# IMMachinations/Task-Vector-Replication

Hardware: AMD Instinct MI355X
Metric: patched-forward prompts/sec, Pythia-2.8B layer×head CIE sweep, 1–8 GPUs (higher is better)
Workload: dtype f32 (x2f16 emulation: fp32 activations as 2 fp16 planes against the checkpoint's exact fp16 weights, 2 MFMA products, fp32 accumulate); 1 GPU; pythia-2.8b CIE sweep 32x32 sites, 12 prompts/step, 4-shot, T=15, fp16-valued weights (exact-fp16 GEMMs, 2 products); parallelism=single GPU, gemm=x2f16, weights=fp16, exact16_gemms=True

## Files before the change

### task-vector-replication_amd/csrc/gemm_pingpong.hpp

```cpp
#pragma once
#include <hip/hip_runtime.h>
#include <stdint.h>

#include <type_traits>

#include "gemm_planar.hpp"

namespace tvr {

constexpr int PP_THREADS = 512;
constexpr int PP_TILE_ELEMS = 256 * 256;

inline int gemm_pingpong_grid(int M, int N) { return ((M + 255) / 256) * ((N + 255) / 256); }

__host__ __device__ inline void pp_tile_coords(int wg, int nbm, int nbn, int& m0, int& n0, int gm = GEMM_GROUP_M) {
  const int per_group = gm * nbn;
  const int grp = wg / per_group;
  const int first_m = grp * gm;
  const int gsz = nbm - first_m < gm ? nbm - first_m : gm;
  const int in_grp = wg - grp * per_group;
  m0 = (first_m + in_grp % gsz) * 256;
  n0 = (in_grp / gsz) * 256;
}

constexpr int PP_EPI_LDR = 260;
#ifndef TVR_PP_NT
#define TVR_PP_NT 1
#endif
constexpr bool PP_NT_STORES = TVR_PP_NT;
#ifndef TVR_PP_SLICE_MIN_K
#define TVR_PP_SLICE_MIN_K 16384
#endif
constexpr int PP_SLICE_MIN_K = TVR_PP_SLICE_MIN_K;
#ifndef TVR_PP_SLICE_FORM
#define TVR_PP_SLICE_FORM 2
#endif
#ifndef TVR_PP_SLICE_FORM_WX
#define TVR_PP_SLICE_FORM_WX 2
#endif
#ifndef TVR_PP_WX_STAGE
#define TVR_PP_WX_STAGE 0
#endif
#ifndef TVR_PP_WX_WIDE
#define TVR_PP_WX_WIDE 2
#endif
#ifndef TVR_PP_BF16_WIDE
#define TVR_PP_BF16_WIDE 0
#endif
#ifndef TVR_PP_WX_2PHASE
#define TVR_PP_WX_2PHASE 0
#endif
#ifndef TVR_PP_PF
#define TVR_PP_PF 1
#endif
__device__ __forceinline__ f32x4 slice_add(f32x4 c, f32x4 t) { return c + t; }
constexpr int PP_EPI_LDS = 128 * PP_EPI_LDR * 2;

template <int CTRL>
__device__ __forceinline__ float dpp_f(float v) {
  return __int_as_float(__builtin_amdgcn_update_dpp(0, __float_as_int(v), CTRL, 0xF, 0xF, false));
}
template <int CTRL>
__device__ __forceinline__ int dpp_i(int v) {
  return __builtin_amdgcn_update_dpp(0, v, CTRL, 0xF, 0xF, false);
}
constexpr int DPP_QUAD_X1 = 0xB1, DPP_QUAD_X2 = 0x4E;
__device__ __forceinline__ void quad_argmax(float& bv, int& bi) {
  argmax_merge(bv, bi, dpp_f<DPP_QUAD_X1>(bv), dpp_i<DPP_QUAD_X1>(bi));
  argmax_merge(bv, bi, dpp_f<DPP_QUAD_X2>(bv), dpp_i<DPP_QUAD_X2>(bi));
}
__device__ __forceinline__ void pp_stats_rows(const GemmEpi& ep, const float* L, int grow0, int col0, int rows,
                                              int Nlim, int t, float acc_scale) {
  const int r = t >> 2, q = t & 3;
  if (r >= rows) return;
  Nlim = min(Nlim, 256);
  const int K = ep.stats_k, rec = 2 + 2 * K, tile = col0 >> 8;
  const float* Lr = L + r * PP_EPI_LDR;
  const float* bias = ep.bias ? ep.bias + col0 : nullptr;
  auto elem = [&](float a, float b) { return __fadd_rn(__fmul_rn(a, acc_scale), b); };
  auto chunk = [&](int i) {
    const int c = 16 * i + 4 * q;
    const f32x4 a = *(const f32x4*)(Lr + c);
    const f32x4 b = bias ? *(const f32x4*)(bias + c) : f32x4{0.f, 0.f, 0.f, 0.f};
    return f32x4{elem(a[0], b[0]), elem(a[1], b[1]), elem(a[2], b[2]), elem(a[3], b[3])};
  };
  const int nc = (Nlim - 4 * q + 15) >> 4;
  float mx = -INFINITY;
#pragma unroll 2
  for (int i = 0; i < nc; ++i) {
    const f32x4 v = chunk(i);
    mx = fmaxf(mx, fmaxf(fmaxf(v[0], v[1]), fmaxf(v[2], v[3])));
  }
  mx = fmaxf(mx, dpp_f<DPP_QUAD_X1>(mx));
  mx = fmaxf(mx, dpp_f<DPP_QUAD_X2>(mx));
  float se = 0.f, bv = -INFINITY;
  int bi = 0x7fffffff;
#pragma unroll 2
  for (int i = 0; i < nc; ++i) {
    const f32x4 v = chunk(i);
    se += (expf(v[0] - mx) + expf(v[1] - mx)) + (expf(v[2] - mx) + expf(v[3] - mx));
#pragma unroll
    for (int e = 0; e < 4; ++e)
      if (v[e] > bv) {
        bv = v[e];
        bi = col0 + 16 * i + 4 * q + e;
      }
  }
  se += dpp_f<DPP_QUAD_X1>(se);
  se += dpp_f<DPP_QUAD_X2>(se);
  const int m = grow0 + r;
  float* o = ep.stats + ((size_t)m * ep.stats_tiles + tile) * rec;
  if (q == 0) {
    o[0] = mx;
    o[1] = se;
    if (ep.targets && ep.tlogit) {
      const int tc = ep.targets[m] - col0;
      if (tc >= 0 && tc < Nlim) ep.tlogit[m] = elem(Lr[tc], bias ? bias[tc] : 0.f);
    }
  }
  for (int j = 0; j < K; ++j) {
    if (j > 0) {
      const float pv = bv;
      const int pi = bi;
      bv = -INFINITY;
      bi = 0x7fffffff;
#pragma unroll 2
  for (int i = 0; i < nc; ++i) {
        const f32x4 v = chunk(i);
#pragma unroll
        for (int e = 0; e < 4; ++e) {
          const int c = col0 + 16 * i + 4 * q + e;
          if ((v[e] < pv || (v[e] == pv && c > pi)) && v[e] > bv) {
            bv = v[e];
            bi = c;
          }
        }
      }
    }
    quad_argmax(bv, bi);
    if (q == 0) {
      o[2 + j] = bv;
      o[2 + K + j] = __int_as_float(bi);
    }
  }
}

template <int EPI, int FMT, bool NOSTORE = false, int TM = 8, int TN = 4>
__device__ __forceinline__ void pp_epilogue_lds(const GemmEpi& ep, const f32x4 (&acc)[TM][TN], float* L, int row0,
                                                int col0, int Mlim, int Nlim, int wr, int wc, int lane, int t,
                                                float acc_scale) {
  static_assert((TM == 8 && TN == 4) || (TM == 4 && TN == 8), "wave tile 128 x 64 or 64 x 128");
  bool split8 = false;
  if constexpr (EPI == EPI_SPLIT_GELU_ACT) split8 = col0 >= ep.n_split && Nlim >= 256;
  float range_mx = 0.f;
  const int c8 = (t & 31) * 8, c4 = (t & 63) * 4;
  float b8[8];
  f32x4 b4 = {0.f, 0.f, 0.f, 0.f};
  if (split8) {
#pragma unroll
    for (int k = 0; k < 8; ++k) b8[k] = ep.bias ? ep.bias[col0 + c8 + k] : 0.f;
  } else if (EPI != EPI_STATS && ep.bias && c4 < Nlim) {
#pragma unroll
    for (int k = 0; k < 4; ++k) b4[k] = ep.bias[col0 + c4 + k];
  }
#pragma unroll
  for (int p = 0; p < 2; ++p) {
    if ((TM == 8 ? wr : wr >> 1) == p) {
      const int r0 = TM == 8 ? 0 : (wr & 1) * 64;
#pragma unroll
      for (int i = 0; i < TM; ++i)
#pragma unroll
        for (int j = 0; j < TN; ++j)
          *(f32x4*)(L + (r0 + i * 16 + (lane & 15)) * PP_EPI_LDR + wc * (16 * TN) + j * 16 + 4 * (lane >> 4)) =
              EPI == EPI_STATS ? acc[i][j] : acc[i][j] * acc_scale;
    }
    __syncthreads();
    const int rows = min(128, Mlim - p * 128);
    if constexpr (EPI == EPI_STATS) {
      pp_stats_rows(ep, L, row0 + p * 128, col0, rows, Nlim, t, acc_scale);
    } else if (split8) {
      constexpr int RPT = 128 / (PP_THREADS / 32);
      const int rb = t >> 5;
      int orow[RPT];
#pragma unroll
      for (int i = 0; i < RPT; ++i) orow[i] = row0 + p * 128 + min(rb + i * (PP_THREADS / 32), max(rows - 1, 0));
      if (ep.out_rows) {
#pragma unroll
        for (int i = 0; i < RPT; ++i) orow[i] = ep.out_rows[orow[i]];
      }
#pragma unroll
      for (int i = 0; i < RPT; ++i) {
        const int r = rb + i * (PP_THREADS / 32);
        if (r >= rows) break;
        const float* src = L + r * PP_EPI_LDR + c8;
        const f32x4 x0 = *(const f32x4*)src, x1 = *(const f32x4*)(src + 4);
        float v[8] = {x0[0] + b8[0], x0[1] + b8[1], x0[2] + b8[2], x0[3] + b8[3],
                      x1[0] + b8[4], x1[1] + b8[5], x1[2] + b8[6], x1[3] + b8[7]};
        const int m = row0 + p * 128 + r;
        if (ep.raw && m < ep.raw_rows) {
          float* q = ep.raw + (size_t)m * ep.ld_raw + (col0 + c8 - ep.n_split);
          *(f32x4*)q = f32x4{v[0], v[1], v[2], v[3]};
          *(f32x4*)(q + 4) = f32x4{v[4], v[5], v[6], v[7]};
        }
#pragma unroll
        for (int k = 0; k < 8; k += 2) {
          const f32x2 g = gelu_erf2(f32x2{v[k], v[k + 1]});
          v[k] = g.x;
          v[k + 1] = g.y;
        }
        if (!NOSTORE || v[0] == 1.2345e-30f)
          store_act8<FMT, PP_NT_STORES>(ep.out1h + (size_t)orow[i] * ep.ld1h + act_col<FMT>(col0 + c8 - ep.n_split),
                                        act_ps<FMT>(ep.ps1h), v,
                                        ep.range_flag, &range_mx);
      }
    } else if (c4 < Nlim) {
      constexpr int RB = 8, NB = 128 / (PP_THREADS / 64) / RB;
      const int rb = t >> 6;
#pragma unroll
      for (int b = 0; b < NB; ++b) {
        int orow[RB];
        f32x4 rr[RB];
#pragma unroll
        for (int i = 0; i < RB; ++i) orow[i] = row0 + p * 128 + min(rb + (b * RB + i) * (PP_THREADS / 64), max(rows - 1, 0));
        if (ep.out_rows) {
#pragma unroll
          for (int i = 0; i < RB; ++i) orow[i] = ep.out_rows[orow[i]];
        }
        if constexpr (EPI == EPI_RESID) {
#pragma unroll
          for (int i = 0; i < RB; ++i) rr[i] = *(const f32x4*)(ep.resid + (size_t)orow[i] * ep.ldr + col0 + c4);
        }
#pragma unroll
        for (int i = 0; i < RB; ++i) {
          const int r = rb + (b * RB + i) * (PP_THREADS / 64);
          if (r >= rows) break;
          f32x4 v = *(const f32x4*)(L + r * PP_EPI_LDR + c4) + b4;
          if (!NOSTORE || v[0] == 1.2345e-30f) {
            if constexpr (EPI == EPI_RESID)
              st16<false>(ep.out0 + (size_t)orow[i] * ep.ld0 + col0 + c4, v + rr[i]);
            else
              epi_store4<EPI, FMT, PP_NT_STORES && EPI == EPI_SPLIT_GELU_ACT>(ep, orow[i], col0 + c4, v);
          }
        }
      }
    }
    __syncthreads();
  }
  if constexpr (EPI == EPI_SPLIT_GELU_ACT && act_is_x2(FMT))
    if (range_mx >= X2_FP16_OVERFLOW && ep.range_flag) atomicOr(ep.range_flag, 1u);
}

template <int FMT>
struct PpLds {
  using F = PlanarFmt<FMT>;
  static constexpr int BUF = 2 * F::NPL * 256 * F::BK;
  static constexpr int HALVES = (2 * BUF + 512) > PP_EPI_LDS ? (2 * BUF + 512) : PP_EPI_LDS;
};

template <int EPI, int FMT, bool VEC, int VAR, bool SL, bool WX = false, bool PFOK = true, bool AIL = false>
__device__ __forceinline__ void pp_tile(const uint16_t* __restrict__ A, int lda, size_t aps,
                                        const uint16_t* __restrict__ W, int ldw, size_t wps, float acc_scale, int M,
                                        int N, const GemmEpi& ep, int m0, int n0, int kbeg, int nk, float* part, int has_part,
                                        unsigned long long st0, unsigned long long sr0) {
  using F = PlanarFmt<FMT>;
  using frag = typename F::frag;
  constexpr int NPL = F::NPL, BK = F::BK, KG = BK / 32;
  constexpr int CPR = BK / 8;
  constexpr int RPP = 64 / CPR;
  constexpr int PPP = 128 / RPP;
  constexpr int PL = 256 * BK;
  static_assert(!WX || FMT == ACT_X2F16, "one-plane weights: x2f16 activations only");
  constexpr int WNPL = WX ? 1 : NPL;
  constexpr int BUF = (NPL + WNPL) * PL;
  constexpr bool P2 = WX && !SL && TVR_PP_WX_2PHASE;
  constexpr int NBUF = P2 ? 3 : 2;
  constexpr int DUMMY = NBUF * BUF;
  constexpr int LDS_HALVES = P2 ? (NBUF * BUF + 512 > PP_EPI_LDS ? NBUF * BUF + 512 : PP_EPI_LDS)
                                : PpLds<FMT>::HALVES;
  static_assert(LDS_HALVES * 2 <= 160 * 1024, "LDS budget (P2)");
  static_assert(NPL * KG == 2, "two fragments per 16-row slice per k-tile");
  static_assert(PpLds<FMT>::HALVES * 2 <= 160 * 1024, "LDS budget");
  static_assert(!AIL || FMT == ACT_X2F16, "the interleaved A layout is an x2f16 form");
  constexpr int ACPR = AIL ? 8 : CPR;
  constexpr int ARPP = 64 / ACPR;
  constexpr int ABK = ACPR * 8;
  constexpr int OFMT = AIL ? (int)ACT_X2F16I : FMT;
  __shared__ __attribute__((aligned(16))) uint16_t lds[LDS_HALVES];

  int t = threadIdx.x;
  asm volatile("" : "+v"(t));
  const int wave = t >> 6, lane = t & 63;
  const int wr = wave >> 2, wc = wave & 3;

  const int wave_s = __builtin_amdgcn_readfirstlane(wave);
  const uint16_t* Ab = ep.a2 != nullptr && n0 >= ep.a2_col ? ep.a2 : A;
  const uint16_t* src[4][2];
  int dst[4][2];
#pragma unroll
  for (int R = 0; R < 4; ++R) {
#pragma unroll
    for (int s = 0; s < 2; ++s) {
      const int pi = (WX && R >= 2) ? wave_s : 2 * wave_s + s;
      const bool ail = AIL && R < 2;
      const int plane = ail ? 0 : pi / PPP;
      const int x0 = ail ? pi * ARPP : (pi % PPP) * RPP;
      int trow0;
      if (R < 2)
        trow0 = ((x0 >> 6) << 7) + (x0 & 63) + 64 * R;
      else
        trow0 = ((x0 >> 5) << 6) + (x0 & 31) + 32 * (R - 2);
      const int row = trow0 + (ail ? lane / ACPR : lane / CPR);
      const int chunk = ail ? (lane % ACPR) ^ planar_g<ACPR>(row) : (lane % CPR) ^ planar_g<CPR>(row);
      if (R < 2) {
        const int am = min(m0 + row, M - 1);
        src[R][s] = Ab + plane * aps + (size_t)(ep.a_rows ? ep.a_rows[am] : am) * lda + chunk * 8;
        dst[R][s] = plane * PL + trow0 * (AIL ? ABK : BK);
      } else {
        src[R][s] = W + plane * wps + (size_t)min(n0 + row, N - 1) * ldw + chunk * 8;
        dst[R][s] = (NPL + plane) * PL + trow0 * BK;
      }
    }
  }
  auto stage = [&](int R, int kt) {
    if (VAR == 1 && kt >= 2) return;
    const bool live = kt < nk;
    const int koff = live && VAR != 12 ? (kbeg + kt) * (AIL && R < 2 ? ABK : BK) : 0;
    const int boff = (P2 ? kt % 3 : kt & 1) * BUF;
#pragma unroll
    for (int s = 0; s < ((WX && R >= 2) ? 1 : 2); ++s) glds16(src[R][s] + koff, lds + (live ? boff + dst[R][s] : DUMMY));
  };

  int aoff[2], boff[2];
#pragma unroll
  for (int f = 0; f < 2; ++f) {
    const int p = NPL == 2 ? f : 0, g = NPL == 2 ? 0 : f;
    const int ra = wr * 128 + (lane & 15), rb = wc * 64 + (lane & 15);
    const int c = 4 * g + (lane >> 4);
    if constexpr (AIL)
      aoff[f] = ra * ABK + (((4 * f + (lane >> 4)) ^ planar_g<ACPR>(ra)) << 3);
    else
      aoff[f] = p * PL + ra * BK + ((c ^ planar_g<CPR>(ra)) << 3);
    boff[f] = (NPL + p) * PL + rb * BK + ((c ^ planar_g<CPR>(rb)) << 3);
  }

  f32x4 acc[8][4];
#pragma unroll
  for (int i = 0; i < 8; ++i)
#pragma unroll
    for (int j = 0; j < 4; ++j) acc[i][j] = f32x4{};
  frag fa[4][2], fwl[2][2], fwh[2][2];
  constexpr bool PF = PFOK && ((TVR_PP_PF != 0) != (VAR == 21)) && !P2 && !WX && !(FMT == ACT_X2F16 && SL);
  [[maybe_unused]] frag fx[2][2];

  const int vi = __builtin_amdgcn_readfirstlane(min(8, max(0, (M - m0 - wr * 128 + 15) >> 4)));
  auto read_a = [&](const uint16_t* base, int i0, auto part, int ifirst = 0) {
#pragma unroll
    for (int i = 0; i < 4; ++i)
      if (i >= ifirst && (!decltype(part)::value || i0 + i < vi))
#pragma unroll
        for (int f = 0; f < 2; ++f) fa[i][f] = *(const frag*)(base + aoff[f] + (i0 + i) * 16 * ABK);
  };
  auto read_fx = [&](const uint16_t* base, auto part) {
#pragma unroll
    for (int i = 0; i < 2; ++i)
      if (!decltype(part)::value || i < vi)
#pragma unroll
        for (int f = 0; f < 2; ++f) fx[i][f] = *(const frag*)(base + aoff[f] + i * 16 * ABK);
  };
  auto read_w = [&](const uint16_t* base, int j0, frag (&fw)[2][2], auto part) {
    if (decltype(part)::value && vi == 0) return;
#pragma unroll
    for (int j = 0; j < 2; ++j)
#pragma unroll
      for (int f = 0; f < (WX ? 1 : 2); ++f) fw[j][f] = *(const frag*)(base + boff[f] + (j0 + j) * 16 * BK);
  };
  [[maybe_unused]] f32x4 tc[2] = {f32x4{0.f, 0.f, 0.f, 0.f}, f32x4{0.f, 0.f, 0.f, 0.f}};
  auto mfma_quadrant = [&](int i0, int j0, const frag (&fw)[2][2], auto part, int ci, int cj) {
#if TVR_PP_SLICE_FORM_WX >= 1
    if constexpr (FMT == ACT_X2F16 && SL && WX && !decltype(part)::value) {
      f32x4 t[4][2];
#pragma unroll
      for (int i = 0; i < 4; ++i) {
        const int di = i == 0 ? ci : i0 + i - 1, dj = i == 0 ? cj : j0;
#pragma unroll
        for (int q = 0; q < 4; ++q) {
          const int j = TVR_PP_SLICE_FORM_WX == 2 ? (q & 1) : (q >> 1), pz = TVR_PP_SLICE_FORM_WX == 2 ? (q >> 1) : (q & 1);
          t[i][j] = __builtin_amdgcn_mfma_f32_16x16x32_f16(fw[j][0], fa[i][pz == 0 ? 1 : 0],
                                                             pz == 0 ? f32x4{0.f, 0.f, 0.f, 0.f} : t[i][j], 0, 0, 0);
          __builtin_amdgcn_sched_group_barrier(0x008, 1, 0);
#pragma unroll
          for (int e = 2 * q; e < 2 * q + 2; ++e)
            acc[di][dj + (e >> 2)][e & 3] += i == 0 ? tc[e >> 2][e & 3] : t[i - 1][e >> 2][e & 3];
          __builtin_amdgcn_sched_group_barrier(0x002, 2, 0);
        }
      }
      tc[0] = t[3][0];
      tc[1] = t[3][1];
      return;
    }
#endif
    if constexpr (FMT == ACT_X2F16 && SL && !WX && !decltype(part)::value) {
#if TVR_PP_SLICE_FORM >= 1
      f32x4 t[4][2];
#pragma unroll
      for (int i = 0; i < 4; ++i) {
        const int di = i == 0 ? ci : i0 + i - 1, dj = i == 0 ? cj : j0;
#pragma unroll
        for (int q = 0; q < 6; ++q) {
          const int j = q & 1, p = q >> 1;
          t[i][j] = __builtin_amdgcn_mfma_f32_16x16x32_f16(fw[j][p == 1 ? 1 : 0], fa[i][p == 0 ? 1 : 0],
                                                             p == 0 ? f32x4{0.f, 0.f, 0.f, 0.f} : t[i][j], 0, 0, 0);
          __builtin_amdgcn_sched_group_barrier(0x008, 1, 0);
#if TVR_PP_SLICE_FORM == 2
          const int e0 = q < 2 ? 0 : 2 * (q - 2), e1 = q < 2 ? 0 : 2 * (q - 2) + 2;
#else
          const int e0 = q < 2 ? 2 * q : q + 2, e1 = q < 2 ? 2 * q + 2 : q + 3;
#endif
#pragma unroll
          for (int e = e0; e < e1; ++e)
            acc[di][dj + (e >> 2)][e & 3] += i == 0 ? tc[e >> 2][e & 3] : t[i - 1][e >> 2][e & 3];
          if (e1 - e0 == 2)
            __builtin_amdgcn_sched_group_barrier(0x002, 2, 0);
          else if (e1 - e0 == 1)
            __builtin_amdgcn_sched_group_barrier(0x002, 1, 0);
        }
      }
      tc[0] = t[3][0];
      tc[1] = t[3][1];
      return;
#else
      (void)ci;
      (void)cj;
      f32x4 t[4][2];
#pragma unroll
      for (int i = 0; i <= 4; ++i) {
        if (i < 4) {
#pragma unroll
          for (int j = 0; j < 2; ++j)
            t[i][j] = __builtin_amdgcn_mfma_f32_16x16x32_f16(fw[j][0], fa[i][1], f32x4{0.f, 0.f, 0.f, 0.f}, 0, 0, 0);
#pragma unroll
          for (int j = 0; j < 2; ++j) t[i][j] = __builtin_amdgcn_mfma_f32_16x16x32_f16(fw[j][1], fa[i][0], t[i][j], 0, 0, 0);
#pragma unroll
          for (int j = 0; j < 2; ++j) t[i][j] = __builtin_amdgcn_mfma_f32_16x16x32_f16(fw[j][0], fa[i][0], t[i][j], 0, 0, 0);
          __builtin_amdgcn_sched_group_barrier(0x008, 6, 0);
        }
        if (i > 0) {
#pragma unroll
          for (int j = 0; j < 2; ++j) acc[i0 + i - 1][j0 + j] = slice_add(acc[i0 + i - 1][j0 + j], t[i - 1][j]);
          __builtin_amdgcn_sched_group_barrier(0x002, 5, 0);
        }
      }
      return;
#endif
    }
#pragma unroll
    for (int i = 0; i < 4; ++i)
#pragma unroll
      for (int j = 0; j < 2; ++j) {
        if (decltype(part)::value && i0 + i >= vi) continue;
        f32x4 c = acc[i0 + i][j0 + j];
        const bool x = PF && i0 == 0 && i < 2;
        const frag a0 = x ? fx[i & 1][0] : fa[i][0], a1 = x ? fx[i & 1][1] : fa[i][1];
        if constexpr (FMT == ACT_X2F16 && SL) {
          f32x4 t = __builtin_amdgcn_mfma_f32_16x16x32_f16(fw[j][0], a1, f32x4{0.f, 0.f, 0.f, 0.f}, 0, 0, 0);
          if constexpr (!WX) t = __builtin_amdgcn_mfma_f32_16x16x32_f16(fw[j][1], a0, t, 0, 0, 0);
          t = __builtin_amdgcn_mfma_f32_16x16x32_f16(fw[j][0], a0, t, 0, 0, 0);
          c = slice_add(c, t);
        } else if constexpr (FMT == ACT_X2F16) {
          c = __builtin_amdgcn_mfma_f32_16x16x32_f16(fw[j][0], a1, c, 0, 0, 0);
          if constexpr (VAR != 15 && !WX)
            c = __builtin_amdgcn_mfma_f32_16x16x32_f16(fw[j][1], a0, c, 0, 0, 0);
          c = __builtin_amdgcn_mfma_f32_16x16x32_f16(fw[j][0], a0, c, 0, 0, 0);
        } else if constexpr (FMT == ACT_F16) {
          c = __builtin_amdgcn_mfma_f32_16x16x32_f16(fw[j][0], a0, c, 0, 0, 0);
          c = __builtin_amdgcn_mfma_f32_16x16x32_f16(fw[j][1], a1, c, 0, 0, 0);
        } else {
          c = __builtin_amdgcn_mfma_f32_16x16x32_bf16(fw[j][0], a0, c, 0, 0, 0);
          c = __builtin_amdgcn_mfma_f32_16x16x32_bf16(fw[j][1], a1, c, 0, 0, 0);
        }
        acc[i0 + i][j0 + j] = c;
      }
  };
  constexpr bool prio = VAR == 14 || (VAR != 2 && VAR != 13 && !(FMT == ACT_X2F16 && SL));
#define TVR_PP_CLUSTER(...)                  \
  __builtin_amdgcn_s_barrier();              \
  __builtin_amdgcn_sched_barrier(0);         \
  if (prio) __builtin_amdgcn_s_setprio(1);   \
  __VA_ARGS__;                               \
  if (prio) __builtin_amdgcn_s_setprio(0);   \
  __builtin_amdgcn_sched_barrier(0);         \
  __builtin_amdgcn_s_barrier();              \
  __builtin_amdgcn_sched_barrier(0)

  constexpr bool XS = WX && TVR_PP_WX_STAGE && !P2;
  if constexpr (P2) {
    stage(0, 0);
    stage(2, 0);
    stage(3, 0);
    stage(1, 0);
    stage(0, 1);
    stage(2, 1);
    stage(3, 1);
    stage(1, 1);
  } else if constexpr (XS) {
    stage(2, 0);
    stage(0, 0);
    stage(3, 0);
    stage(1, 0);
    stage(2, 1);
    stage(0, 1);
  } else {
    stage(0, 0);
    stage(2, 0);
    stage(1, 0);
    stage(3, 0);
    stage(0, 1);
    stage(2, 1);
  }
  if constexpr (P2)
    asm volatile("s_waitcnt vmcnt(8)" ::: "memory");
  else if constexpr (WX)
    asm volatile("s_waitcnt vmcnt(6)" ::: "memory");
  else
    asm volatile("s_waitcnt vmcnt(8)" ::: "memory");
  __builtin_amdgcn_s_barrier();
  __builtin_amdgcn_sched_barrier(0);
  if constexpr (PF) read_fx(lds, std::integral_constant<bool, false>{});
  if (wr == 1 && VAR != 3) {
    __builtin_amdgcn_s_barrier();
    __builtin_amdgcn_sched_barrier(0);
  }

  if (VAR == 13 && wave_s >= 4) __builtin_amdgcn_s_setprio(1);
  unsigned long long d_loop0 = 0, d_loop1 = 0;
  if constexpr (VAR == 6 || VAR == 8) d_loop0 = __builtin_amdgcn_s_memtime();
  auto kloop = [&](auto part) {
    if constexpr (P2) {
      for (int kt = 0; kt < nk; ++kt) {
        const uint16_t* cur = lds + (kt % 3) * BUF;
        read_a(cur, 0, part);
        read_w(cur, 0, fwl, part);
        read_w(cur, 2, fwh, part);
        asm volatile("s_waitcnt vmcnt(6)" ::: "memory");
        stage(0, kt + 2);
        stage(2, kt + 2);
        stage(3, kt + 2);
        TVR_PP_CLUSTER(mfma_quadrant(0, 0, fwl, part, 7, 0); mfma_quadrant(0, 2, fwh, part, 3, 0));
        read_a(cur, 4, part);
        asm volatile("s_waitcnt vmcnt(6)" ::: "memory");
        stage(1, kt + 2);
        TVR_PP_CLUSTER(mfma_quadrant(4, 0, fwl, part, 7, 2); mfma_quadrant(4, 2, fwh, part, 3, 2));
      }
      return;
    }
    for (int kt = 0; kt < nk; ++kt) {
      const uint16_t* cur = lds + (kt & 1) * BUF;
      read_a(cur, 0, part, PF ? 2 : 0);
      read_w(cur, 0, fwl, part);
      if constexpr (XS) {
        asm volatile("s_waitcnt vmcnt(5)" ::: "memory");
        stage(3, kt + 1);
      } else {
        if constexpr (WX) {
          asm volatile("s_waitcnt vmcnt(3)" ::: "memory");
        } else {
          if (VAR != 4) asm volatile("s_waitcnt vmcnt(4)" ::: "memory");
        }
        stage(1, kt + 1);
      }
      TVR_PP_CLUSTER(mfma_quadrant(0, 0, fwl, part, 7, 0));
      read_w(cur, 2, fwh, part);
      if constexpr (XS) {
        asm volatile("s_waitcnt vmcnt(4)" ::: "memory");
        stage(1, kt + 1);
      } else {
        if constexpr (WX) {
          asm volatile("s_waitcnt vmcnt(6)" ::: "memory");
        } else {
          if (VAR != 4) asm volatile("s_waitcnt vmcnt(8)" ::: "memory");
        }
        stage(3, kt + 1);
      }
      TVR_PP_CLUSTER(mfma_quadrant(0, 2, fwh, part, 3, 0));
      read_a(cur, 4, part);
      if constexpr (PF) asm volatile("s_waitcnt vmcnt(6)" ::: "memory");
      stage(XS ? 2 : 0, kt + 2);
      TVR_PP_CLUSTER(mfma_quadrant(4, 2, fwh, part, 3, 2));
      if constexpr (XS) {
        asm volatile("s_waitcnt vmcnt(4)" ::: "memory");
      } else if constexpr (WX) {
        asm volatile("s_waitcnt vmcnt(5)" ::: "memory");
      } else {
        if (VAR != 4) asm volatile("s_waitcnt vmcnt(6)" ::: "memory");
      }
      if constexpr (PF) read_fx(lds + ((kt + 1) & 1) * BUF, part);
      stage(XS ? 0 : 2, kt + 2);
      TVR_PP_CLUSTER(mfma_quadrant(4, 0, fwl, part, 7, 2));
    }
  };
  if (vi == 8) {
    kloop(std::integral_constant<bool, false>{});
#if TVR_PP_SLICE_FORM >= 1
    if constexpr (FMT == ACT_X2F16 && SL && (!WX || TVR_PP_SLICE_FORM_WX >= 1)) {
      acc[7][0] = slice_add(acc[7][0], tc[0]);
      acc[7][1] = slice_add(acc[7][1], tc[1]);
    }
#endif
  } else {
    kloop(std::integral_constant<bool, true>{});
  }
#undef TVR_PP_CLUSTER
  if constexpr (VAR == 6 || VAR == 8) d_loop1 = __builtin_amdgcn_s_memtime();
  if (wr == 0 && VAR != 3) __builtin_amdgcn_s_barrier();
  asm volatile("s_waitcnt vmcnt(0)" ::: "memory");

  if constexpr (VEC && VAR != 7) {
    __syncthreads();
    float* L = reinterpret_cast<float*>(lds);
    if (has_part) {
      GemmEpi pe = ep;
      pe.out0 = part;
      pe.ld0 = 256;
      pe.out_rows = nullptr;
      pp_epilogue_lds<EPI, OFMT, VAR == 8>(pe, acc, L, 0, 0, M - m0, N - n0, wr, wc, lane, t, acc_scale);
    } else {
      pp_epilogue_lds<EPI, OFMT, VAR == 8>(ep, acc, L, m0, n0, M - m0, N - n0, wr, wc, lane, t, acc_scale);
    }
    if ((VAR == 6 || VAR == 8) && ep.stamps && t == 0) {
      unsigned long long* o = ep.stamps + 4 * blockIdx.x;
      o[0] = st0;
      o[1] = d_loop0;
      o[2] = d_loop1;
      o[3] = __builtin_amdgcn_s_memtime();
    }
    return;
  }
  if constexpr (EPI == EPI_STATS) {
    return;
  } else {
    if (acc_scale != 1.0f) {
#pragma unroll
      for (int i = 0; i < 8; ++i)
#pragma unroll
        for (int j = 0; j < 4; ++j) acc[i][j] *= acc_scale;
    }
    if (has_part) {
      GemmEpi pe = ep;
      pe.out0 = part;
      pe.ld0 = 256;
      gemm_epilogue16t<EPI, OFMT, VEC, 8, 4>(pe, acc, M - m0, N - n0, wr * 128, wc * 64, lane);
    } else {
      gemm_epilogue16t<EPI, OFMT, VEC, 8, 4>(ep, acc, M, N, m0 + wr * 128, n0 + wc * 64, lane);
    }
    if (VAR == 6 && ep.stamps && t == 0) {
      unsigned long long* o = ep.stamps + 4 * blockIdx.x;
      o[0] = st0;
      o[1] = d_loop0;
      o[2] = d_loop1;
      o[3] = __builtin_amdgcn_s_memtime();
    } else if (ep.stamps && t == 0) {
      ep.stamps[2 * blockIdx.x] = __builtin_amdgcn_s_memtime() - st0;
      ep.stamps[2 * blockIdx.x + 1] = __builtin_amdgcn_s_memrealtime() - sr0;
    }
  }
}

#ifndef TVR_WT_SGB
#define TVR_WT_SGB 1
#endif
template <int EPI, int FMT, bool VEC, int VAR, bool SL, bool TWO = false, bool AIL = false, bool WIL = false>
__device__ __forceinline__ void pp_tile_wt(const uint16_t* __restrict__ A, int lda, size_t aps,
                                           const uint16_t* __restrict__ W, int ldw, float acc_scale, int M, int N,
                                           const GemmEpi& ep, int m0, int n0, int kbeg, int nk, float* part,
                                           int has_part, unsigned long long st0, unsigned long long sr0) {
  using F = PlanarFmt<FMT>;
  using frag = typename F::frag;
  constexpr int NPL = F::NPL;
  constexpr int BK = F::BK;
  constexpr int KG = BK / 32;
  constexpr int CPR = BK / 8;
  constexpr int RPP = 64 / CPR;
  constexpr int PPP = 128 / RPP;
  constexpr int WP = PPP / 8;
  constexpr int PL = 256 * BK;
  constexpr int BUF = (NPL + 1) * PL;
  constexpr int NBUF = TWO ? 3 : 2;
  static_assert(!TWO || FMT == ACT_X2F16, "three 64 KB bf16 buffers do not fit the LDS");
  static_assert(NPL * KG == 2, "two A fragments per 16-row tile per k-tile");
  static_assert(!SL || FMT == ACT_X2F16, "the sliced accumulation is an x2f16 form");
  static_assert(!AIL || FMT == ACT_X2F16, "the interleaved A layout is an x2f16 form");
  constexpr int ACPR = AIL ? 8 : CPR;
  constexpr int ARPP = 64 / ACPR;
  constexpr int ABK = ACPR * 8;
  constexpr int VM = 4 + 2 * WP, VM0 = 4 + 3 * WP;
  constexpr int DUMMY = NBUF * BUF;
  constexpr int LDS_HALVES = (NBUF * BUF + 512) > PP_EPI_LDS ? (NBUF * BUF + 512) : PP_EPI_LDS;
  static_assert(LDS_HALVES * 2 <= 160 * 1024, "LDS budget");
  __shared__ __attribute__((aligned(16))) uint16_t lds[LDS_HALVES];
  constexpr int OFMT = AIL ? (int)ACT_X2F16I : FMT;

  int t = threadIdx.x;
  asm volatile("" : "+v"(t));
  const int wave = t >> 6, lane = t & 63;
  const int wr = wave >> 1, wc = wave & 1;
  const int wave_s = __builtin_amdgcn_readfirstlane(wave);
  const uint16_t* Ab = ep.a2 != nullptr && n0 >= ep.a2_col ? ep.a2 : A;

  const uint16_t* src[4][2];
  int dst[4][2];
#pragma unroll
  for (int R = 0; R < 4; ++R) {
#pragma unroll
    for (int s = 0; s < 2; ++s) {
      const int pi = R >= 2 ? WP * wave_s + (WP > 1 ? s : 0) : 2 * wave_s + s;
      const bool ail = AIL && R < 2;
      const int plane = ail ? 0 : pi / PPP;
      const int x0 = ail ? pi * ARPP : (pi % PPP) * RPP;
      const int trow0 = R < 2 ? ((x0 >> 5) << 6) + (x0 & 31) + 32 * R : ((x0 >> 6) << 7) + (x0 & 63) + 64 * (R - 2);
      const int row = trow0 + (ail ? lane / ACPR : lane / CPR);
      const int chunk = ail ? (lane % ACPR) ^ planar_g<ACPR>(row) : (lane % CPR) ^ planar_g<CPR>(row);
      if (R < 2) {
        const int am = min(m0 + row, M - 1);
        src[R][s] = Ab + plane * aps + (size_t)(ep.a_rows ? ep.a_rows[am] : am) * lda + chunk * 8;
        dst[R][s] = plane * PL + trow0 * (AIL ? ABK : BK);
      } else {
        const int wn = min(n0 + row, N - 1);
        if constexpr (WIL)
          src[R][s] = W + (size_t)(wn >> 1) * (2 * ldw) + (wn & 1) * 32 + chunk * 8;
        else
          src[R][s] = W + (size_t)wn * ldw + chunk * 8;
        dst[R][s] = NPL * PL + trow0 * BK;
      }
    }
  }
  auto stage = [&](int R, int kt) {
    const bool live = kt < nk;
    const int koff = live ? (kbeg + kt) * ((AIL && R < 2) || (WIL && R >= 2) ? 64 : BK) : 0;
    const int boff = (TWO ? kt % 3 : kt & 1) * BUF;
#pragma unroll
    for (int s = 0; s < (R >= 2 ? WP : 2); ++s) glds16(src[R][s] + koff, lds + (live ? boff + dst[R][s] : DUMMY));
  };

  int aoff[2], woff[KG];
#pragma unroll
  for (int f = 0; f < 2; ++f) {
    const int p = NPL == 2 ? f : 0, g = NPL == 2 ? 0 : f;
    const int ra = wr * 64 + (lane & 15), c = 4 * g + (lane >> 4);
    if constexpr (AIL)
      aoff[f] = ra * ABK + (((4 * f + (lane >> 4)) ^ planar_g<ACPR>(ra)) << 3);
    else
      aoff[f] = p * PL + ra * BK + ((c ^ planar_g<CPR>(ra)) << 3);
  }
#pragma unroll
  for (int g = 0; g < KG; ++g) {
    const int rb = wc * 128 + (lane & 15), c = 4 * g + (lane >> 4);
    woff[g] = NPL * PL + rb * BK + ((c ^ planar_g<CPR>(rb)) << 3);
  }

  f32x4 acc[4][8];
#pragma unroll
  for (int i = 0; i < 4; ++i)
#pragma unroll
    for (int j = 0; j < 8; ++j) acc[i][j] = f32x4{};
  frag fa[4][2], fw[8][KG];

  const int vi = __builtin_amdgcn_readfirstlane(min(4, max(0, (M - m0 - wr * 64 + 15) >> 4)));
  auto read_a = [&](const uint16_t* base, int i0, auto part) {
#pragma unroll
    for (int i = i0; i < i0 + 2; ++i)
      if (!decltype(part)::value || i < vi)
#pragma unroll
        for (int f = 0; f < 2; ++f) fa[i][f] = *(const frag*)(base + aoff[f] + i * 16 * ABK);
  };
  auto read_w = [&](const uint16_t* base, int j0, auto part) {
    if (decltype(part)::value && vi == 0) return;
#pragma unroll
    for (int j = j0; j < j0 + 4; ++j)
#pragma unroll
      for (int g = 0; g < KG; ++g) fw[j][g] = *(const frag*)(base + woff[g] + j * 16 * BK);
  };
  [[maybe_unused]] f32x4 tc[2] = {f32x4{0.f, 0.f, 0.f, 0.f}, f32x4{0.f, 0.f, 0.f, 0.f}};
  constexpr int NJ = TWO ? 8 : 4, NP = NJ / 2;
  auto cluster = [&](int i0, int j0, auto part, int ci, int cj) {
    if constexpr (SL && !decltype(part)::value) {
      f32x4 s[2][2];
#pragma unroll
      for (int q = 0; q < 2 * NP; ++q) {
        const int i = i0 + q / NP, j = j0 + 2 * (q % NP);
        const int pi = q == 0 ? ci : i0 + (q - 1) / NP, pj = q == 0 ? cj : j0 + 2 * ((q - 1) % NP);
#pragma unroll
        for (int u = 0; u < 4; ++u) {
          const int jj = u & 1, pz = u >> 1;
          s[q & 1][jj] = __builtin_amdgcn_mfma_f32_16x16x32_f16(fw[j + jj][0], fa[i][pz == 0 ? 1 : 0],
                                                                 pz == 0 ? f32x4{0.f, 0.f, 0.f, 0.f} : s[q & 1][jj],
                                                                 0, 0, 0);
          if (TVR_WT_SGB) __builtin_amdgcn_sched_group_barrier(0x008, 1, 0);
#pragma unroll
          for (int e = 2 * u; e < 2 * u + 2; ++e)
            acc[pi][pj + (e >> 2)][e & 3] += q == 0 ? tc[e >> 2][e & 3] : s[(q - 1) & 1][e >> 2][e & 3];
          if (TVR_WT_SGB) __builtin_amdgcn_sched_group_barrier(0x002, 2, 0);
        }
        if (NP == 4 && q == NP - 1) __builtin_amdgcn_sched_barrier(0);
      }
      tc[0] = s[(2 * NP - 1) & 1][0];
      tc[1] = s[(2 * NP - 1) & 1][1];
      return;
    }
#pragma unroll
    for (int i = i0; i < i0 + 2; ++i)
#pragma unroll
      for (int j = j0; j < j0 + NJ; ++j) {
        if (decltype(part)::value && i >= vi) continue;
        f32x4 c = acc[i][j];
        if constexpr (SL) {
          f32x4 s = __builtin_amdgcn_mfma_f32_16x16x32_f16(fw[j][0], fa[i][1], f32x4{0.f, 0.f, 0.f, 0.f}, 0, 0, 0);
          s = __builtin_amdgcn_mfma_f32_16x16x32_f16(fw[j][0], fa[i][0], s, 0, 0, 0);
          c = slice_add(c, s);
        } else if constexpr (FMT == ACT_X2F16) {
          c = __builtin_amdgcn_mfma_f32_16x16x32_f16(fw[j][0], fa[i][1], c, 0, 0, 0);
          c = __builtin_amdgcn_mfma_f32_16x16x32_f16(fw[j][0], fa[i][0], c, 0, 0, 0);
        } else if constexpr (FMT == ACT_F16) {
          c = __builtin_amdgcn_mfma_f32_16x16x32_f16(fw[j][0], fa[i][0], c, 0, 0, 0);
          c = __builtin_amdgcn_mfma_f32_16x16x32_f16(fw[j][KG - 1], fa[i][1], c, 0, 0, 0);
        } else {
          c = __builtin_amdgcn_mfma_f32_16x16x32_bf16(fw[j][0], fa[i][0], c, 0, 0, 0);
          c = __builtin_amdgcn_mfma_f32_16x16x32_bf16(fw[j][KG - 1], fa[i][1], c, 0, 0, 0);
        }
        acc[i][j] = c;
      }
  };
  constexpr bool prio = !SL;
#define TVR_PP_CLUSTER(...)                  \
  __builtin_amdgcn_s_barrier();              \
  __builtin_amdgcn_sched_barrier(0);         \
  if (prio) __builtin_amdgcn_s_setprio(1);   \
  __VA_ARGS__;                               \
  if (prio) __builtin_amdgcn_s_setprio(0);   \
  __builtin_amdgcn_sched_barrier(0);         \
  __builtin_amdgcn_s_barrier();              \
  __builtin_amdgcn_sched_barrier(0)

  if constexpr (TWO) {
#pragma unroll
    for (int k = 0; k < 2; ++k) {
      stage(0, k);
      stage(2, k);
      stage(1, k);
      stage(3, k);
    }
    asm volatile("s_waitcnt vmcnt(6)" ::: "memory");
  } else {
    stage(0, 0);
    stage(2, 0);
    stage(3, 0);
    stage(1, 0);
    stage(0, 1);
    stage(2, 1);
    stage(3, 1);
    asm volatile("s_waitcnt vmcnt(%0)" ::"n"(VM0) : "memory");
  }
  __builtin_amdgcn_s_barrier();
  __builtin_amdgcn_sched_barrier(0);
  if (vi == 4)
    read_a(lds, 0, std::integral_constant<bool, false>{});
  else
    read_a(lds, 0, std::integral_constant<bool, true>{});
  if (wr >= 2) {
    __builtin_amdgcn_s_barrier();
    __builtin_amdgcn_sched_barrier(0);
  }
  unsigned long long d_loop0 = 0, d_loop1 = 0;
  if constexpr (VAR == 6 || VAR == 8) d_loop0 = __builtin_amdgcn_s_memtime();
  auto kloop = [&](auto part) {
    if constexpr (TWO) {
      for (int kt = 0; kt < nk; ++kt) {
        const uint16_t* cur = lds + (kt % 3) * BUF;
        read_w(cur, 0, part);
        read_w(cur, 4, part);
        asm volatile("s_waitcnt vmcnt(4)" ::: "memory");
        stage(0, kt + 2);
        stage(2, kt + 2);
        TVR_PP_CLUSTER(cluster(0, 0, part, 3, 6));
        read_a(cur, 2, part);
        read_a(lds + ((kt + 1) % 3) * BUF, 0, part);
        asm volatile("s_waitcnt vmcnt(3)" ::: "memory");
        stage(1, kt + 2);
        stage(3, kt + 2);
        TVR_PP_CLUSTER(cluster(2, 0, part, 1, 6));
      }
      return;
    }
    for (int kt = 0; kt < nk; ++kt) {
      const uint16_t* cur = lds + (kt & 1) * BUF;
      read_w(cur, 0, part);
      asm volatile("s_waitcnt vmcnt(%0)" ::"n"(VM) : "memory");
      stage(1, kt + 1);
      TVR_PP_CLUSTER(cluster(0, 0, part, 3, 2));
      read_w(cur, 4, part);
      asm volatile("s_waitcnt vmcnt(%0)" ::"n"(VM) : "memory");
      stage(0, kt + 2);
      TVR_PP_CLUSTER(cluster(0, 4, part, 1, 2));
      read_a(cur, 2, part);
      asm volatile("s_waitcnt vmcnt(%0)" ::"n"(VM) : "memory");
      stage(2, kt + 2);
      TVR_PP_CLUSTER(cluster(2, 4, part, 1, 6));
      read_a(lds + ((kt + 1) & 1) * BUF, 0, part);
      asm volatile("s_waitcnt vmcnt(%0)" ::"n"(VM) : "memory");
      stage(3, kt + 2);
      TVR_PP_CLUSTER(cluster(2, 0, part, 3, 6));
    }
  };
  if (vi == 4) {
    kloop(std::integral_constant<bool, false>{});
    if constexpr (SL) {
      acc[3][TWO ? 6 : 2] = slice_add(acc[3][TWO ? 6 : 2], tc[0]);
      acc[3][TWO ? 7 : 3] = slice_add(acc[3][TWO ? 7 : 3], tc[1]);
    }
  } else {
    kloop(std::integral_constant<bool, true>{});
  }
#undef TVR_PP_CLUSTER
  if constexpr (VAR == 6 || VAR == 8) d_loop1 = __builtin_amdgcn_s_memtime();
  if (wr < 2) __builtin_amdgcn_s_barrier();
  asm volatile("s_waitcnt vmcnt(0)" ::: "memory");

  if constexpr (VEC) {
    __syncthreads();
    float* L = reinterpret_cast<float*>(lds);
    if (has_part) {
      GemmEpi pe = ep;
      pe.out0 = part;
      pe.ld0 = 256;
      pe.out_rows = nullptr;
      pp_epilogue_lds<EPI, OFMT, VAR == 8, 4, 8>(pe, acc, L, 0, 0, M - m0, N - n0, wr, wc, lane, t, acc_scale);
    } else {
      pp_epilogue_lds<EPI, OFMT, VAR == 8, 4, 8>(ep, acc, L, m0, n0, M - m0, N - n0, wr, wc, lane, t, acc_scale);
    }
    if ((VAR == 6 || VAR == 8) && ep.stamps && t == 0) {
      unsigned long long* o = ep.stamps + 4 * blockIdx.x;
      o[0] = st0;
      o[1] = d_loop0;
      o[2] = d_loop1;
      o[3] = __builtin_amdgcn_s_memtime();
    }
    return;
  }
  if constexpr (EPI == EPI_STATS) {
    return;
  } else {
    if (acc_scale != 1.0f) {
#pragma unroll
      for (int i = 0; i < 4; ++i)
#pragma unroll
        for (int j = 0; j < 8; ++j) acc[i][j] *= acc_scale;
    }
    if (has_part) {
      GemmEpi pe = ep;
      pe.out0 = part;
      pe.ld0 = 256;
      gemm_epilogue16t<EPI, OFMT, VEC, 4, 8>(pe, acc, M - m0, N - n0, wr * 64, wc * 128, lane);
    } else {
      gemm_epilogue16t<EPI, OFMT, VEC, 4, 8>(ep, acc, M, N, m0 + wr * 64, n0 + wc * 128, lane);
    }
    if (ep.stamps && t == 0) {
      ep.stamps[2 * blockIdx.x] = __builtin_amdgcn_s_memtime() - st0;
      ep.stamps[2 * blockIdx.x + 1] = __builtin_amdgcn_s_memrealtime() - sr0;
    }
  }
}

template <int EPI, int FMT, bool VEC, int VAR, bool SL, bool WX, bool SKM, bool AIL = false, bool WIL = false>
__device__ __forceinline__ void pp_tile_any(const uint16_t* __restrict__ A, int lda, size_t aps,
                                            const uint16_t* __restrict__ W, int ldw, size_t wps, float acc_scale,
                                            int M, int N, const GemmEpi& ep, int m0, int n0, int kbeg, int nk,
                                            float* part, int has_part, unsigned long long st0,
                                            unsigned long long sr0) {
  constexpr bool wide = (WX && FMT == ACT_X2F16 &&
                         (VAR == 16 || VAR == 20 || (VAR != 17 && TVR_PP_WX_WIDE && (VAR == 0 || VAR == 6 || VAR == 8)))) ||
                        ((FMT == ACT_BF16 || FMT == ACT_F16) &&
                         (VAR == 16 || (VAR != 17 && TVR_PP_BF16_WIDE && (VAR == 0 || VAR == 6 || VAR == 8))));
  constexpr bool two = FMT == ACT_X2F16 && (VAR == 20 || (VAR != 16 && TVR_PP_WX_WIDE == 2 && !SL));
  constexpr int V = (VAR == 16 || VAR == 17 || VAR == 20) ? 0 : VAR;
  static_assert(!AIL || FMT == ACT_X2F16, "the interleaved A layout is an x2f16 form");
  static_assert(!WIL || wide, "the interleaved weight plane: the wide one-plane tile only");
  if constexpr (wide)
    pp_tile_wt<EPI, FMT, VEC, V, SL, two, AIL, WIL>(A, lda, aps, W, ldw, acc_scale, M, N, ep, m0, n0, kbeg, nk, part, has_part,
                                          st0, sr0);
  else
    pp_tile<EPI, FMT, VEC, V, SL, WX, !SKM && EPI != EPI_STATS, AIL>(A, lda, aps, W, ldw, wps, acc_scale, M, N, ep, m0, n0,
                                                                kbeg, nk, part, has_part, st0, sr0);
}

template <int EPI, int FMT, bool VEC = true, int VAR = 0, bool SKM = false, bool SL = false, bool WX = false,
          bool AIL = false, bool WIL = false>
__global__ void __launch_bounds__(PP_THREADS, 1)
gemm_pingpong_kernel(const uint16_t* __restrict__ A, int lda, size_t aps, const uint16_t* __restrict__ W, int ldw,
                     size_t wps, float acc_scale, int M, int N, int K, GemmEpi ep) {
  const unsigned long long st0 = ep.stamps ? __builtin_amdgcn_s_memtime() : 0;
  const unsigned long long sr0 = ep.stamps ? __builtin_amdgcn_s_memrealtime() : 0;
  const int nbm = (M + 255) >> 8, nbn = (N + 255) >> 8;
  const int nk_all = K / PlanarFmt<FMT>::BK;
  const int gm = ep.group_m > 0 ? ep.group_m : GEMM_GROUP_M;
  auto remap = [](int bid, int nwg) {
    const int xcd = bid & 7, q = nwg >> 3, r = nwg & 7;
    return (xcd < r ? xcd * (q + 1) : r * (q + 1) + (xcd - r) * q) + (bid >> 3);
  };
  const int count = ep.tile_count > 0 ? ep.tile_count : nbm * nbn;
  if constexpr (SKM) {
    const int G = ep.sk_blocks;
    const int g = remap(blockIdx.x, G);
    const long long I = (long long)count * nk_all;
    long long it = (long long)g * I / G;
    const long long it1 = (long long)(g + 1) * I / G;
    auto segment = [&](int seg) {
      const int lt = (int)(it / nk_all);
      const int kbeg = (int)(it - (long long)lt * nk_all);
      const int nk = (int)min((long long)(nk_all - kbeg), it1 - it);
      int m0, n0;
      pp_tile_coords(ep.tile_base + lt, nbm, nbn, m0, n0, gm);
      pp_tile_any<EPI, FMT, VEC, VAR, SL, WX, SKM, AIL, WIL>(A, lda, aps, W, ldw, wps, acc_scale, M, N, ep, m0, n0, kbeg, nk,
                                  ep.out0 + ((size_t)2 * g + seg) * PP_TILE_ELEMS, 1, st0, sr0);
      it += nk;
    };
    segment(0);
    if (it < it1) segment(1);
  } else {
    const int S = ep.k_split > 1 ? ep.k_split : 1;
    const int wgs = remap(blockIdx.x, count * S);
    const int lt = wgs / S, split = wgs - lt * S;
    int m0, n0;
    pp_tile_coords(ep.tile_base + lt, nbm, nbn, m0, n0, gm);
    const int kbeg = (int)((long long)split * nk_all / S);
    const int nk = (int)((long long)(split + 1) * nk_all / S) - kbeg;
    pp_tile_any<EPI, FMT, VEC, VAR, SL, WX, SKM, AIL, WIL>(A, lda, aps, W, ldw, wps, acc_scale, M, N, ep, m0, n0, kbeg, nk,
                                ep.out0 + ((size_t)split * count + lt) * PP_TILE_ELEMS, S > 1, st0, sr0);
  }
}

template <int EPI, int FMT>
__global__ void __launch_bounds__(256)
splitk_reduce_kernel(const float* __restrict__ part, int S, int tile_base, int count, int M, int N, GemmEpi ep) {
  const int nbm = (M + 255) >> 8, nbn = (N + 255) >> 8;
  const size_t total = (size_t)count * (PP_TILE_ELEMS / 4);
  for (size_t i = blockIdx.x * (size_t)blockDim.x + threadIdx.x; i < total; i += (size_t)gridDim.x * blockDim.x) {
    const int lt = (int)(i / (PP_TILE_ELEMS / 4)), e = (int)(i % (PP_TILE_ELEMS / 4)) * 4;
    int m0, n0;
    pp_tile_coords(tile_base + lt, nbm, nbn, m0, n0, ep.group_m > 0 ? ep.group_m : GEMM_GROUP_M);
    const int m = m0 + (e >> 8), c = n0 + (e & 255);
    if (m >= M || c >= N) continue;
    const float* p = part + (size_t)lt * PP_TILE_ELEMS + e;
    f32x4 v = *(const f32x4*)p;
    for (int s = 1; s < S; ++s) v += *(const f32x4*)(p + (size_t)s * count * PP_TILE_ELEMS);
    if (ep.bias) {
#pragma unroll
      for (int r = 0; r < 4; ++r) v[r] += ep.bias[c + r];
    }
    const size_t orow = ep.out_rows ? (size_t)ep.out_rows[m] : (size_t)m;
    epi_store4<EPI, FMT>(ep, orow, c, v);
  }
}

template <int EPI, int FMT>
__global__ void __launch_bounds__(256)
splitk_sk_reduce_kernel(const float* __restrict__ part, int G, int KT, int tile_base, int count, int M, int N,
                        GemmEpi ep) {
  const int nbm = (M + 255) >> 8, nbn = (N + 255) >> 8;
  const long long I = (long long)count * KT;
  const size_t total = (size_t)count * (PP_TILE_ELEMS / 4);
  for (size_t i = blockIdx.x * (size_t)blockDim.x + threadIdx.x; i < total; i += (size_t)gridDim.x * blockDim.x) {
    const int lt = (int)(i / (PP_TILE_ELEMS / 4)), e = (int)(i % (PP_TILE_ELEMS / 4)) * 4;
    int m0, n0;
    pp_tile_coords(tile_base + lt, nbm, nbn, m0, n0, ep.group_m > 0 ? ep.group_m : GEMM_GROUP_M);
    const int m = m0 + (e >> 8), c = n0 + (e & 255);
    if (m >= M || c >= N) continue;
    const long long x0 = (long long)lt * KT, x1 = x0 + KT - 1;
    const int b0 = (int)(((x0 + 1) * G - 1) / I), b1 = (int)(((x1 + 1) * G - 1) / I);
    f32x4 v = {0.f, 0.f, 0.f, 0.f};
    for (int b = b0; b <= b1; ++b) {
      const int slot = ((long long)b * I / G) < x0 ? 1 : 0;
      v += *(const f32x4*)(part + ((size_t)2 * b + slot) * PP_TILE_ELEMS + e);
    }
    if (ep.bias) {
#pragma unroll
      for (int r = 0; r < 4; ++r) v[r] += ep.bias[c + r];
    }
    const size_t orow = ep.out_rows ? (size_t)ep.out_rows[m] : (size_t)m;
    epi_store4<EPI, FMT>(ep, orow, c, v);
  }
}


inline int pp_ktile(int fmt) { return fmt == ACT_X2F16 ? PlanarFmt<ACT_X2F16>::BK : PlanarFmt<ACT_BF16>::BK; }
static_assert(PlanarFmt<ACT_F16>::BK == PlanarFmt<ACT_BF16>::BK, "pp_ktile: fp16 and bf16 share a k-tile length");

inline bool pp_sliced_rule(int K, int K2) { return K >= PP_SLICE_MIN_K || K2 >= PP_SLICE_MIN_K; }

struct PpForm {
  int epi, fmt;
  bool vec, skm, sl, wx, ail;
};
using PpKernel = void (*)(const uint16_t*, int, size_t, const uint16_t*, int, size_t, float, int, int, int, GemmEpi);

constexpr bool pp_form_exists(int epi, int fmt, bool vec, bool skm, bool sl, bool wx, bool ail) {
  if (fmt != ACT_X2F16 && (sl || wx || ail)) return false;
  if (ail && !wx && (epi != EPI_BIAS || skm)) return false;
  if (skm) return epi == EPI_BIAS && vec;
  switch (epi) {
    case EPI_BIAS: return true;
    case EPI_SPLIT_GELU_ACT:
    case EPI_RESID: return fmt != ACT_F16;
    case EPI_STATS: return fmt != ACT_F16 && vec;
    default: return false;
  }
}

template <int EPI, int FMT, bool VEC, bool SKM, bool SL, bool WX, bool AIL>
PpKernel pp_kernel_at() {
  if constexpr (pp_form_exists(EPI, FMT, VEC, SKM, SL, WX, AIL))
    return gemm_pingpong_kernel<EPI, FMT, VEC, 0, SKM, SL, WX, AIL>;
  else
    return nullptr;
}
template <int EPI, int FMT, bool... B, class... Rest>
PpKernel pp_kernel_at(bool b, Rest... rest) {
  return b ? pp_kernel_at<EPI, FMT, B..., true>(rest...) : pp_kernel_at<EPI, FMT, B..., false>(rest...);
}
template <int EPI>
PpKernel pp_kernel_epi(const PpForm& f) {
  switch (f.fmt) {
    case ACT_X2F16: return pp_kernel_at<EPI, ACT_X2F16>(f.vec, f.skm, f.sl, f.wx, f.ail);
    case ACT_BF16: return pp_kernel_at<EPI, ACT_BF16>(f.vec, f.skm, f.sl, f.wx, f.ail);
    case ACT_F16: return pp_kernel_at<EPI, ACT_F16>(f.vec, f.skm, f.sl, f.wx, f.ail);
    default: return nullptr;
  }
}
template <int VAR = 0>
PpKernel pp_kernel(const PpForm& f) {
  static_assert(VAR == 0, "the engine's forms run VAR 0");
  switch (f.epi) {
    case EPI_BIAS: return pp_kernel_epi<EPI_BIAS>(f);
    case EPI_SPLIT_GELU_ACT: return pp_kernel_epi<EPI_SPLIT_GELU_ACT>(f);
    case EPI_RESID: return pp_kernel_epi<EPI_RESID>(f);
    case EPI_STATS: return pp_kernel_epi<EPI_STATS>(f);
    default: return nullptr;
  }
}

inline int pp_reduce_fmt(int a_fmt, bool ail) { return ail ? ACT_X2F16I : a_fmt == ACT_X2F16 ? ACT_X2F16 : ACT_BF16; }
using PpReduceKernel = void (*)(const float*, int, int, int, int, int, GemmEpi);
using PpSkReduceKernel = void (*)(const float*, int, int, int, int, int, int, GemmEpi);
template <bool SK, int EPI, int FMT>
auto pp_reduce_at() {
  if constexpr (SK)
    return PpSkReduceKernel(splitk_sk_reduce_kernel<EPI, FMT>);
  else
    return PpReduceKernel(splitk_reduce_kernel<EPI, FMT>);
}
template <bool SK, int EPI>
auto pp_reduce_epi(int out_fmt) -> decltype(pp_reduce_at<SK, EPI, ACT_BF16>()) {
  switch (out_fmt) {
    case ACT_X2F16I: return pp_reduce_at<SK, EPI, ACT_X2F16I>();
    case ACT_X2F16: return pp_reduce_at<SK, EPI, ACT_X2F16>();
    case ACT_BF16: return pp_reduce_at<SK, EPI, ACT_BF16>();
    default: return nullptr;
  }
}
template <bool SK>
auto pp_reduce_kernel(int epi, int out_fmt) -> decltype(pp_reduce_at<SK, EPI_BIAS, ACT_BF16>()) {
  switch (epi) {
    case EPI_BIAS: return pp_reduce_epi<SK, EPI_BIAS>(out_fmt);
    case EPI_SPLIT_GELU_ACT: return pp_reduce_epi<SK, EPI_SPLIT_GELU_ACT>(out_fmt);
    case EPI_RESID: return pp_reduce_epi<SK, EPI_RESID>(out_fmt);
    default: return nullptr;
  }
}

}
```

Baseline: 19740 patched prompts/s.

## Add direct-to-global GELU epilogue by permuting weight rows in the pingpong GEMM

For full-width split-GELU tiles with the interleaved x2f16 output format, the weight rows loaded into LDS are permuted so that each lane's accumulator fragment maps to eight contiguous output columns. Each lane then applies bias and GELU and stores directly to global memory, skipping the LDS staging round trip and the barrier before the epilogue. It also records extra realtime stamps when stamping is enabled. The risk is more register pressure in the epilogue and stores that are less coalesced than the LDS-staged path.

```diff
diff --git a/task-vector-replication_amd/csrc/gemm_pingpong.hpp b/task-vector-replication_amd/csrc/gemm_pingpong.hpp
--- a/task-vector-replication_amd/csrc/gemm_pingpong.hpp
+++ b/task-vector-replication_amd/csrc/gemm_pingpong.hpp
@@ -248,6 +248,60 @@
   }
   if constexpr (EPI == EPI_SPLIT_GELU_ACT && act_is_x2(FMT))
     if (range_mx >= X2_FP16_OVERFLOW && ep.range_flag) atomicOr(ep.range_flag, 1u);
+}
+
+#ifndef TVR_PP_DIRECT
+#define TVR_PP_DIRECT 1
+#endif
+__host__ __device__ constexpr int pp_direct_wrow(int r) {
+  return (r & ~31) | (((r >> 2) & 3) << 3) | (((r >> 4) & 1) << 2) | (r & 3);
+}
+template <int FMT, bool NOSTORE = false>
+__device__ __forceinline__ void pp_epilogue_direct(const GemmEpi& ep, const f32x4 (&acc)[4][8], int row0, int col0,
+                                                   int Mlim, int wr, int wc, int lane, float acc_scale) {
+  static_assert(FMT == ACT_X2F16I, "a lane's 8 columns are one 16-B piece of each plane's half line");
+  const int rl = wr * 64 + (lane & 15), cl = wc * 128 + 8 * (lane >> 4);
+  float b[4][8];
+#pragma unroll
+  for (int J = 0; J < 4; ++J)
+#pragma unroll
+    for (int k = 0; k < 8; ++k) b[J][k] = ep.bias ? ep.bias[col0 + cl + 32 * J + k] : 0.f;
+  int orow[4];
+#pragma unroll
+  for (int i = 0; i < 4; ++i) orow[i] = row0 + min(rl + 16 * i, Mlim - 1);
+  if (ep.out_rows) {
+#pragma unroll
+    for (int i = 0; i < 4; ++i) orow[i] = ep.out_rows[orow[i]];
+  }
+  float range_mx = 0.f;
+#pragma unroll
+  for (int i = 0; i < 4; ++i) {
+    if (rl + 16 * i >= Mlim) continue;
+    const int m = row0 + rl + 16 * i;
+#pragma unroll
+    for (int J = 0; J < 4; ++J) {
+      const int c = col0 + cl + 32 * J - ep.n_split;
+      float v[8];
+#pragma unroll
+      for (int k = 0; k < 8; ++k)
+        v[k] = __fadd_rn(__fmul_rn(acc[i][2 * J + (k >> 2)][k & 3], acc_scale), b[J][k]);
+      if (ep.raw && m < ep.raw_rows) {
+        float* q = ep.raw + (size_t)m * ep.ld_raw + c;
+        *(f32x4*)q = f32x4{v[0], v[1], v[2], v[3]};
+        *(f32x4*)(q + 4) = f32x4{v[4], v[5], v[6], v[7]};
+      }
+#pragma unroll
+      for (int k = 0; k < 8; k += 2) {
+        const f32x2 g = gelu_erf2(f32x2{v[k], v[k + 1]});
+        v[k] = g.x;
+        v[k + 1] = g.y;
+      }
+      if (!NOSTORE || v[0] == 1.2345e-30f)
+        store_act8<FMT, PP_NT_STORES>(ep.out1h + (size_t)orow[i] * ep.ld1h + act_col<FMT>(c), act_ps<FMT>(ep.ps1h), v,
+                                      ep.range_flag, &range_mx);
+    }
+  }
+  if (range_mx >= X2_FP16_OVERFLOW && ep.range_flag) atomicOr(ep.range_flag, 1u);
 }
 
 template <int FMT>
@@ -705,6 +759,9 @@
   const int wr = wave >> 1, wc = wave & 1;
   const int wave_s = __builtin_amdgcn_readfirstlane(wave);
   const uint16_t* Ab = ep.a2 != nullptr && n0 >= ep.a2_col ? ep.a2 : A;
+  constexpr bool DIRECT = TVR_PP_DIRECT && VEC && EPI == EPI_SPLIT_GELU_ACT && OFMT == ACT_X2F16I && !WIL;
+  bool direct = false;
+  if constexpr (DIRECT) direct = !has_part && n0 >= ep.n_split && N - n0 >= 256;
 
   const uint16_t* src[4][2];
   int dst[4][2];
@@ -724,7 +781,7 @@
         src[R][s] = Ab + plane * aps + (size_t)(ep.a_rows ? ep.a_rows[am] : am) * lda + chunk * 8;
         dst[R][s] = plane * PL + trow0 * (AIL ? ABK : BK);
       } else {
-        const int wn = min(n0 + row, N - 1);
+        const int wn = min(n0 + (direct ? pp_direct_wrow(row) : row), N - 1);
         if constexpr (WIL)
           src[R][s] = W + (size_t)(wn >> 1) * (2 * ldw) + (wn & 1) * 32 + chunk * 8;
         else
@@ -925,9 +982,11 @@
   asm volatile("s_waitcnt vmcnt(0)" ::: "memory");
 
   if constexpr (VEC) {
-    __syncthreads();
+    if (!direct) __syncthreads();
     float* L = reinterpret_cast<float*>(lds);
-    if (has_part) {
+    if (direct) {
+      if constexpr (DIRECT) pp_epilogue_direct<OFMT, VAR == 8>(ep, acc, m0, n0, M - m0, wr, wc, lane, acc_scale);
+    } else if (has_part) {
       GemmEpi pe = ep;
       pe.out0 = part;
       pe.ld0 = 256;
@@ -942,6 +1001,9 @@
       o[1] = d_loop0;
       o[2] = d_loop1;
       o[3] = __builtin_amdgcn_s_memtime();
+      unsigned long long* r = ep.stamps + 4 * (size_t)gridDim.x + 2 * blockIdx.x;
+      r[0] = sr0;
+      r[1] = __builtin_amdgcn_s_memrealtime();
     }
     return;
   }
```

Measured after the change: 19780 patched prompts/s, median of 4. No clear change (+0.2%).
